# ztlpn/minilp

Measured on AMD Instinct MI355X. Metric: simplex pivots/sec, higher is better.
Workload: dtype f64; 1 GPU; config 4: random LP 100000 vars x 100000 constraints, 100 nnz/row (0.1% fill), Max c'x, Ax<=b, x>=0; primal simplex with PSE+DSE from the slack basis; timed pivots 5..1983; parallelism=1 GPU, nucleus_size_at_end=1559, completed_steps=1978

## Files before the change

include/minilp_hip.h:

```cpp
#ifndef MINILP_HIP_H
#define MINILP_HIP_H

#include <stdint.h>

#ifdef __cplusplus
extern "C" {
#endif

typedef struct mlp_problem mlp_problem;
typedef struct mlp_solution mlp_solution;

enum { MLP_MINIMIZE = 0, MLP_MAXIMIZE = 1 };
enum { MLP_EQ = 0, MLP_LE = 1, MLP_GE = 2 };
enum { MLP_OK = 0, MLP_INFEASIBLE = 1, MLP_UNBOUNDED = 2,
       MLP_EINVAL = -1, MLP_ESINGULAR = -2, MLP_EHIP = -3, MLP_ENOGPU = -4, MLP_ENOMEM = -5 };

#define MLP_ABI_VERSION 5u
uint32_t mlp_abi_version(void);
uint64_t mlp_stats_size(void);

const char* mlp_last_error(void);
int mlp_device_count(void);
int mlp_set_device(int device);

// ... 185 lines not shown
    int32_t phase;
    int32_t next_stage;
    int32_t reserved;
    int64_t col, row;
    int64_t entering_var, leaving_var;
    double pivot_coeff;
    double step;
    double objective;
    uint64_t nucleus_size;
} mlp_iter_info;
int mlp_engine_open(mlp_solution* s, mlp_iter_info* out);
int mlp_engine_stage(mlp_solution* s, int stage, mlp_iter_info* out);

double mlp_util_min_cut(uint32_t n, const double* weights, uint8_t* side_out);

#ifdef __cplusplus
}
#endif
#endif
```

minilp_amd/api.py:

```python
import ctypes as C
import os

import numpy as np

_HERE = os.path.dirname(os.path.abspath(__file__))
_SO = os.path.join(_HERE, "libminilp_hip.so")
os.environ.setdefault("HSA_ENABLE_IPC_MODE_LEGACY", "0")

MINIMIZE, MAXIMIZE = 0, 1
EQ, LE, GE = 0, 1, 2


class Infeasible(Exception):
    pass


class Unbounded(Exception):
    pass


class InternalError(Exception):
    def __init__(self, code, msg):
        super().__init__(f"[{code}] {msg}")
        self.code = code
# ... 131 lines not shown
    sig("mlp_solution_add_gomory_cut", i32, C.POINTER(vp), u32)
    sig("mlp_solution_stats", None, vp, C.POINTER(MlpStats))
    sig("mlp_solution_reset_stats", None, vp)
    sig("mlp_solution_trace_len", u64, vp)
    sig("mlp_solution_trace_get", None, vp, u64, C.POINTER(C.c_int32), C.POINTER(i64), C.POINTER(i64), C.POINTER(i64),
        C.POINTER(i64), pdbl, pdbl)
    sig("mlp_solution_state", u64, vp, C.c_char_p, pdbl, u64)
    sig("mlp_mps_parse", i32, C.c_char_p, u64, i32, C.POINTER(vp))
    sig("mlp_mps_free", None, vp)
    sig("mlp_mps_name", C.c_char_p, vp)
    sig("mlp_mps_num_vars", u32, vp)
    sig("mlp_mps_var_name", C.c_char_p, vp, u32)
    sig("mlp_mps_var_index", i64, vp, C.c_char_p)
    sig("mlp_mps_problem", vp, vp)
    sig("mlp_util_min_cut", C.c_double, u32, pdbl, C.POINTER(C.c_uint8))
    sig("mlp_solution_num_constraints", u64, vp)
    sig("mlp_solution_dual_values", i32, vp, pdbl, u64)
    sig("mlp_solution_dual_value", i32, vp, u64, pdbl)
    sig("mlp_solution_reduced_costs", i32, vp, pdbl, u32)
    sig("mlp_solution_reduced_cost", i32, vp, u32, pdbl)
    sig("mlp_solution_certificate", i32, vp, C.POINTER(MlpCertificate))
    sig("mlp_ranging_info_size", u64)
    if L.mlp_ranging_info_size() != C.sizeof(MlpRangingInfo):
        raise ImportError(f"{_SO}: mlp_ranging_info is {L.mlp_ranging_info_size()} bytes, this binding {C.sizeof(MlpRangingInfo)}: rebuild it")
    sig("mlp_solution_basis_status", i32, vp, C.POINTER(C.c_int32), u32, C.POINTER(C.c_int32), u64)
    sig("mlp_solution_cost_ranging", i32, vp, pu32, u64, pdbl, pdbl)
    sig("mlp_solution_rhs_ranging", i32, vp, C.POINTER(C.c_uint64), u64, pdbl, pdbl)
    sig("mlp_solution_ranging_info", i32, vp, C.POINTER(MlpRangingInfo))
    sig("mlp_cut_info_size", u64)
    if L.mlp_cut_info_size() != C.sizeof(MlpCutInfo):
# ... 79 lines not shown
    return idx, val


def _p(a, t):
    return a.ctypes.data_as(C.POINTER(t))


def min_cut(weights):
    w = np.ascontiguousarray(weights, dtype=np.float64)
    n = w.shape[0]
    side = np.zeros(n, dtype=np.uint8)
    val = lib().mlp_util_min_cut(n, _p(w, C.c_double), _p(side, C.c_uint8))
    return float(val), side.astype(bool)


class Problem:

    def __init__(self, direction, _h=None):
        self._h = _h if _h is not None else lib().mlp_problem_new(int(direction))
        self.direction = direction

    def __del__(self):
        if getattr(self, "_h", None):
            lib().mlp_problem_free(self._h)
            self._h = None

    def clone(self):
        return Problem(self.direction, lib().mlp_problem_clone(self._h))

    @property
# ... 425 lines not shown
```

minilp_amd/csrc/capi.hip:

```cpp
#include "../../include/minilp_hip.h"

#include <cmath>
#include <cstring>
#include <string>
#include <vector>

#include "engine.h"

using namespace mlp;


struct mlp_problem {
    ProblemData pd;
};
struct mlp_solution {
    Engine* eng = nullptr;
    bool duals_valid = false;
    Engine::Duals duals;
    Engine::RangingInfo ranging;
    Engine::CutInfo cuts;
    Engine::TableauInfo tableau;
    Engine::GmiInfo gmi;
    std::vector<uint64_t> tab_indptr;
    std::vector<uint32_t> tab_indices;
// ... 608 lines not shown
    s->eng->stats = Stats();
    s->eng->restart_sampling();
}
uint64_t mlp_solution_trace_len(const mlp_solution* s) { return s->eng->trace_log.size(); }
void mlp_solution_trace_get(const mlp_solution* s, uint64_t i, int32_t* phase, int64_t* col, int64_t* row,
                            int64_t* entering_var, int64_t* leaving_var, double* pivot_coeff, double* obj_after) {
    const PivotRecord& r = s->eng->trace_log[i];
    *phase = r.phase; *col = r.col; *row = r.row; *entering_var = r.entering_var; *leaving_var = r.leaving_var;
    *pivot_coeff = r.pivot_coeff; *obj_after = r.obj_after;
}
uint64_t mlp_solution_state(const mlp_solution* s, const char* what, double* out, uint64_t cap) {
    uint64_t n = (uint64_t)-1;
    guarded([&] { n = s->eng->state(what, out, cap); });
    return n;
}

int mlp_mps_parse(const char* text, uint64_t len, int direction, mlp_mps** out) {
    *out = nullptr;
    mlp_mps* f = new mlp_mps();
    int st = guarded([&] { f->d = parse_mps(std::string(text, len), direction == MLP_MAXIMIZE ? 1 : 0); });
    if (st != 0) delete f;
    else *out = f;
    return st;
}
void mlp_mps_free(mlp_mps* f) { delete f; }
const char* mlp_mps_name(const mlp_mps* f) { return f->d.name.c_str(); }
uint32_t mlp_mps_num_vars(const mlp_mps* f) { return (uint32_t)f->d.var_names.size(); }
const char* mlp_mps_var_name(const mlp_mps* f, uint32_t i) { return f->d.var_names[i].c_str(); }
int64_t mlp_mps_var_index(const mlp_mps* f, const char* name) {
    for (size_t i = 0; i < f->d.var_names.size(); ++i)
// ... 11 lines not shown
```

minilp_amd/csrc/engine.h:

```cpp
#pragma once
#include <hip/hip_runtime.h>

#include <cstdint>
#include <functional>
#include <utility>
#include <stdexcept>
#include <string>
#include <vector>

#include "kernels.h"

namespace mlp {

enum Stage { STAGE_FTRAN = 0, STAGE_RATIO = 1, STAGE_BTRAN = 2, STAGE_BASIS = 3, STAGE_ROW = 4, STAGE_APPLY = 5 };

struct MlpError : std::runtime_error {
    int code;
    MlpError(int c, const std::string& s) : std::runtime_error(s), code(c) {}
};
struct LpFail {
    int code;
};

#define HIPCHECK(expr)                                                                                   \
// ... 308 lines not shown
    DevBuf<unsigned char> d_pk_valid;
    DevBuf<unsigned char> d_fmark;
    bool use_pack = true;
    bool pack_built = false;
    size_t band_total_ = 0;
    bool use_order = true;
    uint64_t order_built_at = 0;
    uint64_t lifetime_pivots = 0;
    uint64_t order_every = 2048;
    bool order_valid = false;
    uint64_t order_from = 4096;
    bool order_force = false;
    void refresh_nb_order(bool force);
    int det_mode = -1;
    int banded_mode = -1;
    bool use_banded() const;
  public:
    bool banded_active() const { return use_banded(); }
    bool factor_active() const { return fac_on_; }
    void restart_sampling() { batches_run = 0; }
  private:
    void ensure_banded();
    DevBuf<int> d_fpk_cnt, d_fpk_var;
    DevBuf<double> d_fpk_val, d_fpk_x, d_fpk_part;
    DevBuf<unsigned char> d_fpk_in;
    bool fpull_on_ = true;
    bool fpk_valid_ = false;
    uint64_t fpk_built_at_ = 0, fpk_builds_ = 0;
    int fpk_every_ = 1024;
    bool fpk_wanted() const;
// ... 156 lines not shown
```

minilp_amd/csrc/engine.hip:

```cpp
#include "engine.h"


#include <algorithm>
#include <chrono>
#include <cmath>
#include <cstdio>
#include <cstdlib>
#include <climits>
#include <cstring>
#include <limits>
#include <map>
#include <memory>
#include <mutex>

#include <dlfcn.h>
#include <fcntl.h>
#include <sys/mman.h>
#include <sys/stat.h>
#include <unistd.h>

namespace mlp {

static const double INF = std::numeric_limits<double>::infinity();
static double now_s() {
// ... 39 lines not shown
    std::memset(&hview, 0, sizeof(hview));
    const char* ng = std::getenv("MLP_NO_GRAPH");
    use_graph = !(ng && ng[0] == '1');
    const char* rt = std::getenv("MLP_REFRESH_TOL");
    if (rt) refresh_tol = std::atof(rt);
    const char* lr = std::getenv("MLP_LOWRANK");
    if (lr) lr_force = std::max(0, std::min(LR_MAX, std::atoi(lr)));
    const char* lp = std::getenv("MLP_LDPAD");
    if (lp) ld_pad = std::max(0, std::min(4096, std::atoi(lp))) & ~1;
    const char* bt = std::getenv("MLP_BIGTILE");
    force_big_tiles = bt && std::atoi(bt) != 0;
    const char* dm = std::getenv("MLP_DETERMINISTIC");
    if (dm) det_mode = std::atoi(dm) != 0 ? 1 : 0;
    const char* bd = std::getenv("MLP_BANDED");
    if (bd) banded_mode = std::atoi(bd) != 0 ? 1 : 0;
    const char* fr = std::getenv("MLP_FINAL_REFRESH");
    if (fr) final_refresh_pivots = std::atol(fr);
    if (const char* sp = std::getenv("MLP_SWEEP_PACKED")) use_pack = sp[0] != '0';
    if (const char* of = std::getenv("MLP_ORDER_FROM")) order_from = (uint64_t)std::atoll(of);
    if (const char* oe = std::getenv("MLP_ORDER_EVERY")) order_every = (uint64_t)std::atoll(oe);
    const char* lz = std::getenv("MLP_LAZY_DSE");
    lazy_dse = !(lz && lz[0] == '0');
    ratio_two = std::getenv("MLP_RATIO_TWO_KERNELS") != nullptr;
    if (const char* hy = std::getenv("MLP_HYPER")) hyper_mode = std::atoi(hy) > 0 ? 1 : 0;
    if (const char* phk = std::getenv("MLP_PRIMAL_HEAD_K")) ph_kmax = std::max(0, std::atoi(phk));
    if (const char* sbk = std::getenv("MLP_SMALL_BASIS_K")) sb_kmax = std::max(0, std::min(256, std::atoi(sbk)));
    if (const char* sk = std::getenv("MLP_STR_K")) str_kmax = std::atoi(sk);
    if (const char* hh = std::getenv("MLP_HYPER_HEAVY")) hyper_heavy = std::atol(hh);
    if (const char* rs = std::getenv("MLP_RATIO_SPIN_LIMIT")) ratio_spin_limit = std::atoll(rs);
    if (const char* sb = std::getenv("MLP_STREAM_BALANCED")) sw_balanced = std::atoi(sb);
// ... 212 lines not shown
    const int lr = lr_force >= 0 ? lr_force : (cap_ >= 8192 ? 32 : 0);
    g.head_fused = (!fac_on_ && lr == 0 && max_col_nnz_ <= HEAD_LIST_CAP && max_row_nnz_ <= HEAD_LIST_CAP) ? 1 : 0;
    g.fac = fac_on_ ? 1 : 0;
    g.ratio_two = (ratio_two || (shard_world > 1 && ranks_share_device)) ? 1 : 0;
    g.ratio_list = ratio_spin_limit > 0 ? 1 : 0;
    g.str = (str_now && !stepping && !fac_on_) ? 1 : 0;
    g.sb = (g.str && sb_now) ? 1 : 0;
    g.ph = (g.str && ph_now) ? 1 : 0;
    g.fp = hview.fpk_on ? 1 : 0;
    return g;
}

bool Engine::use_banded() const {
    if (banded_mode == 0) return false;
    if (banded_mode == 1) return true;
    return m_ >= 4 * BAND_ROWS && h_rcol.size() >= ((size_t)1 << 22);
}
void Engine::ensure_banded() {
    if (!banded_dirty) return;
    const int nb = (m_ + BAND_ROWS - 1) / BAND_ROWS;
    const size_t np = (size_t)nb * (size_t)(N_ + 1);
    d_bptr.ensure(np, 0, st);
    d_scan_tmp.ensure(np / 4096 + 8, 0, st);
    launch_band_count(d_cptr.p, d_crow.p, N_, nb, d_bptr.p, st);
    launch_exclusive_scan(d_bptr.p, d_bptr.p, (long)np, d_scan_tmp.p, st);
    int total = 0;
    HIPCHECK(hipMemcpyAsync(&total, d_scan_tmp.p + (np + 4095) / 4096, sizeof(int), hipMemcpyDeviceToHost, st));
    HIPCHECK(hipStreamSynchronize(st));
    d_brow.ensure((size_t)total + 8, 0, st);
    d_bval.ensure((size_t)total + 8, 0, st);
    band_total_ = (size_t)total;
    pack_built = false;
    HIPCHECK(hipMemsetAsync(d_brow.p + total, 0, 8 * sizeof(unsigned short), st));
    HIPCHECK(hipMemsetAsync(d_bval.p + total, 0, 8 * sizeof(double), st));
    launch_band_fill(d_cptr.p, d_crow.p, d_cval.p, N_, nb, d_bptr.p, d_brow.p, d_bval.p, st);
    d_band_part.ensure((size_t)nb * (size_t)num_vars, 0, st);
    banded_dirty = false;
}

void Engine::refresh_nb_order(bool force) {
    if (!force && (!order_valid || lifetime_pivots - order_built_at < order_every)) return;
    std::vector<int> ord;
    ord.reserve((size_t)num_vars);
    for (int var = 0; var < N_; ++var)
        if (h_var_loc[var] < 0) ord.push_back(-1 - h_var_loc[var]);
    if ((int)ord.size() != num_vars) throw MlpError(-3, "refresh_nb_order: host mirror of var_loc is inconsistent");
    d_nb_order.ensure((size_t)num_vars, 0, st);
    HIPCHECK(hipMemcpyAsync(d_nb_order.p, ord.data(), sizeof(int) * (size_t)num_vars, hipMemcpyHostToDevice, st));
    HIPCHECK(hipStreamSynchronize(st));
    order_built_at = lifetime_pivots;
    order_valid = true;
    pack_built = false;
    if (use_pack && band_total_ > 0 && !banded_dirty) {
        const int nb = (m_ + BAND_ROWS - 1) / BAND_ROWS;
        const size_t np = (size_t)nb * ((size_t)num_vars + 1);
        try {
            d_pk_ptr.ensure(np, 0, st);
            {
                const unsigned short* r0 = d_pk_row.p;
                const double* v0 = d_pk_val.p;
                d_pk_row.ensure(band_total_ + 16, 0, st);
                d_pk_val.ensure(band_total_ + 16, 0, st);
                if (d_pk_row.p != r0) HIPCHECK(hipMemsetAsync(d_pk_row.p, 0, sizeof(unsigned short) * d_pk_row.cap, st));
                if (d_pk_val.p != v0) HIPCHECK(hipMemsetAsync(d_pk_val.p, 0, sizeof(double) * d_pk_val.cap, st));
            }
            d_pk_valid.ensure((size_t)num_vars, 0, st);
            d_scan_tmp.ensure(np / 4096 + 8, 0, st);
        } catch (MlpError&) {
            (void)hipGetLastError();
// ... 87 lines not shown
    v.det_pull = (!v.pb_on && (det_mode == 1 || shard_det || force_det_push_ || (det_mode < 0 && h_rcol.size() <= ((size_t)1 << 21)))) ? 1 : 0;
    if (v.det_pull) {
        const unsigned char* before = d_fmark.p;
        d_fmark.ensure((size_t)m_ + 64, 0, st);
        if (d_fmark.p != before) HIPCHECK(hipMemsetAsync(d_fmark.p, 0, d_fmark.cap, st));
        v.fmark = d_fmark.p;
    } else {
        v.fmark = nullptr;
    }
    v.banded = use_banded() ? 1 : 0;
    if (v.banded) ensure_banded();
    v.bptr = v.banded ? d_bptr.p : nullptr;
    v.brow = v.banded ? d_brow.p : nullptr;
    v.bval = v.banded ? d_bval.p : nullptr;
    v.band_part = v.banded ? d_band_part.p : nullptr;
    v.nbands = (m_ + BAND_ROWS - 1) / BAND_ROWS;
    if (v.banded && use_order && shard_world == 1 && (lifetime_pivots >= order_from || order_force)) {
        if (!order_valid || (use_pack && !pack_built)) refresh_nb_order(true);
        v.nb_order = d_nb_order.p;
    } else {
        v.nb_order = nullptr;
    }
    const bool pk = v.nb_order && use_pack && pack_built;
    v.pk_ptr = pk ? d_pk_ptr.p : nullptr; v.pk_row = pk ? d_pk_row.p : nullptr; v.pk_val = pk ? d_pk_val.p : nullptr;
    v.pk_valid = pk ? d_pk_valid.p : nullptr;
    v.pos_of_kslot = d_pos_of_kslot.p; v.row_of_kslot = d_row_of_kslot.p; v.W = d_W.p;
    v.U = d_U.p; v.V = d_V.p; v.Ut = d_Ut.p;
    v.lrJ = fac_on_ ? 0 : (lr_force >= 0 ? lr_force : (cap_ >= 8192 ? 32 : 0));
    v.alpha_q = d_work.p;
    v.tau = d_work.p + (size_t)m_;
    v.rv = reinterpret_cast<double2*>(d_work.p + 2 * (size_t)m_);
// ... 2696 lines not shown
    e->h_obj = h_obj; e->h_lo = h_lo; e->h_hi = h_hi; e->h_rhs = h_rhs;
    e->h_cons_row = h_cons_row;
    e->h_rptr = h_rptr; e->h_rcol = h_rcol; e->h_rval = h_rval;
    e->h_colnnz = h_colnnz; e->h_single_row = h_single_row; e->h_single_val = h_single_val;
    e->max_col_nnz_ = max_col_nnz_; e->max_row_nnz_ = max_row_nnz_; e->amax_ = amax_; e->fpull_on_ = fpull_on_;
    e->sw_balanced = sw_balanced; e->str_kmax = str_kmax; e->sb_kmax = sb_kmax; e->ph_kmax = ph_kmax; e->hyper_mode = hyper_mode; e->hyper_heavy = hyper_heavy; e->hyper_backoff_max = hyper_backoff_max; e->ratio_two = ratio_two; e->ratio_spin_limit = ratio_spin_limit; e->ranks_share_device = false; e->lazy_dse = lazy_dse; e->beta_stale = beta_stale; e->use_order = use_order; e->use_pack = use_pack; e->order_force = order_force; e->lifetime_pivots = lifetime_pivots;
    e->h_basic_vars = h_basic_vars; e->h_nb_vars = h_nb_vars; e->h_var_loc = h_var_loc;
    e->h_kslot_of_pos = h_kslot_of_pos; e->h_srow_of_pos = h_srow_of_pos; e->h_kslot_of_row = h_kslot_of_row;
    e->h_pos_of_srow = h_pos_of_srow; e->h_sdiag_of_pos = h_sdiag_of_pos; e->h_nb_fixed = h_nb_fixed;
    e->h_pos_of_kslot = h_pos_of_kslot; e->h_row_of_kslot = h_row_of_kslot;
    e->enable_pse = enable_pse; e->enable_dse = enable_dse;
    e->primal_feasible = primal_feasible; e->dual_feasible = dual_feasible;
    e->resume_in_optimize = resume_in_optimize;
    e->nnz_nonbasic = nnz_nonbasic;
    e->trace = trace; e->profile = profile;
    e->banded_mode = banded_mode; e->det_mode = det_mode;
    e->final_refresh_pivots = final_refresh_pivots; e->iters_since_recalc = iters_since_recalc;
    e->iters_since_polish = iters_since_polish;
    e->ld_pad = ld_pad; e->lr_force = lr_force; e->force_big_tiles = force_big_tiles;
    hipStream_t s2 = e->st;
    {
        const size_t nz = h_rcol.size();
        e->d_cptr.copy_from(d_cptr, (size_t)N_ + 1, s2); e->d_crow.copy_from(d_crow, nz, s2); e->d_cval.copy_from(d_cval, nz, s2);
        e->d_rptr.copy_from(d_rptr, (size_t)m_ + 1, s2); e->d_rcol.copy_from(d_rcol, nz, s2); e->d_rval.copy_from(d_rval, nz, s2);
        e->d_lo.copy_from(d_lo, (size_t)N_, s2); e->d_hi.copy_from(d_hi, (size_t)N_, s2); e->d_obj.copy_from(d_obj, (size_t)N_, s2);
        e->colblk_dirty = true;
        e->banded_dirty = true;
        e->view_dirty = true;
    }
    int mk = m_;
    e->m_ = 0;
// ... 80 lines not shown
    else if (w == "dev_csc_indices") from_dev_i(d_crow, h_rcol.size());
    else if (w == "dev_csc_data") from_dev_d(d_cval.p, h_rcol.size());
    else if (w == "dev_csr_indptr") from_dev_i(d_rptr, (size_t)m_ + 1);
    else if (w == "dev_csr_data") from_dev_d(d_rval.p, h_rcol.size());
    else if (w == "flags") tmp = {(double)primal_feasible, (double)dual_feasible, (double)enable_pse, (double)enable_dse};
    else if (w == "small_basis_launches") {
        pull_ctl();
        tmp = {(double)h_ctl->sb_count};
    } else if (w == "dual_list_tests") {
        int n_ = 0, p_ = 0;
        HIPCHECK(hipMemcpy(&n_, &d_ctl.p->ar_used, sizeof(int), hipMemcpyDeviceToHost));
        HIPCHECK(hipMemcpy(&p_, &d_ctl.p->ar_pauses, sizeof(int), hipMemcpyDeviceToHost));
        tmp = {(double)n_, (double)p_};
    } else if (w == "fpull") {
        tmp = {(double)(hview.fpk_on ? 1 : 0), (double)fpk_builds_, (double)fpk_built_at_, (double)(fpull_supported(hview, geom()) ? 1 : 0)};
    } else if (w == "ratio_primal_form") {
        tmp = {(double)ratio_primal_form(hview, geom())};
    } else if (w == "ratio_list") {
        pull_ctl();
        const Geom g_ = geom();
        tmp = {(double)((ratio_primal_form(hview, g_) == 1 && ratio_list_cap(hview, g_) >= 0) ? 1 : 0), (double)h_ctl->rl_decisions, (double)h_ctl->rl_overflows};
    } else if (w == "btran_ride") {
        pull_ctl();
        tmp = {(double)(btran_rides_ratio(hview, geom()) ? 1 : 0), (double)h_ctl->rk_rides};
    } else if (w == "golive_checks") {
        tmp = {(double)golive_checks_};
    } else if (w == "shard_live") {
        tmp = {(double)(shard_is_live() ? 1 : 0)};
    } else if (w == "primal_head_launches") {
        pull_ctl();
// ... 492 lines not shown
```

minilp_amd/csrc/kernels.h:

```cpp
#pragma once
#include <hip/hip_runtime.h>
#include <stdint.h>

namespace mlp {

constexpr double EPS = 1e-8;

enum IterStatus : int {
    ITER_PIVOT = 0,
    ITER_FLIP = 1,
    ITER_OPTIMAL = 2,
    ITER_UNBOUNDED = 3,
    ITER_FEASIBLE = 4,
    ITER_INFEASIBLE = 5,
    ITER_SINGULAR = 6,
    ITER_NONE = 7,
    ITER_COMM = 8,
    ITER_STALL = 9,
};

struct IterState {
    int status;
    int q;
    int r;
// ... 161 lines not shown
    int* srow_of_pos;
    double* sdiag_of_pos;
    int* kslot_of_row;
    int* pos_of_srow;
    RowInfo* rowinfo;
    int* colblk;
    double* push_part;
    int pb_rb, pb_on;
    int pb_det, pb_hbits;
    double pb_amax;
    int* bptr;
    unsigned short* brow;
    double* bval;
    double2* band_part;
    int nbands, banded;
    unsigned char* fmark;
    int det_pull;
    int* pos_of_kslot;
    int* row_of_kslot;
    double* W;
    double* U;
    double* Ut;
    double* V;
    int lrJ;
    int sw_nbal, sw_pad;
    int* hy_stamp_n;
    int* hy_stamp_p;
    int* hy_var_slot;
    int2* hy_brng;
    double* hy_score;
// ... 70 lines not shown
};
constexpr int FAC_BMAX = 1024;
constexpr int AR_CAP = 2048;
constexpr int RK_LDS = 64;
constexpr int RL_CAP = 8;
constexpr int RL_BLOCKS = 512;
constexpr int TK_ONE = 128;
constexpr int TK_GROUPS = 16;
constexpr int TK_STRIDE = 1024;
constexpr int TK_WORDS = TK_STRIDE * (TK_GROUPS + 1) + 8;
constexpr int FAC_BAR_FLAG = TK_WORDS + 1024;

constexpr int FW_TR = 8;
constexpr int FW_TC = 1024;

constexpr int BAND_ROWS = 8192;
constexpr int BAND_THREADS = 1024;
constexpr int PB_ROWS = 4096;
constexpr int PB_CHUNKS = 48;
constexpr int PB_CHUNKS_DEFAULT = 24;

struct Geom {
    int m, n, cap;
    int lanes;
    int sweep_one;
    int sweep_variant;
    int big;
    int head_fused;
    int str;
    int sb;
    int fac;
// ... 149 lines not shown
    double2* rv;
    int k, fac;
};
int tab_wt_stripes(int k);
void launch_tab_rows(const DevView& dv, const Geom& g, const RangingBufs& b, int nreq, const int* h_req, double* ad, int* cnt, int* off,
                     int* sums, int* len, double* rhs, hipStream_t st);
void launch_tab_rhs(const DevView& dv, const TabBufs& b, const int* req, int nreq, int mode, hipStream_t st);
void launch_tab_solve(const DevView& dv, const Geom& g, const TabBufs& b, int transpose, int nreq, hipStream_t st);
void launch_blocked_inverse(const DevView& dv, int k, double* rowbuf, int nrowbuf, int* piv, int* src, double* prow, double* ckey,
                            int* cidx, int* flag, hipStream_t st);

void launch_csc_append_rows(const int* optr, const int* orow, const double* oval, int n_old, int row0, int R, const int* rptr,
                            const int* rcol, const double* rval, int* cnt, int* sums, int* nptr, int* nrow, double* nval,
                            hipStream_t st);
void launch_exclusive_scan(const int* in, int* out, long n, int* sums, hipStream_t st);
void launch_band_count(const int* cptr, const int* crow, int N, int nbands, int* cnt, hipStream_t st);
void launch_pack_count(const DevView& dv, int* cnt, hipStream_t st);
void launch_pack_fill(const DevView& dv, const int* pkptr, unsigned short* prow, double* pval, unsigned char* valid, hipStream_t st);
void launch_band_fill(const int* cptr, const int* crow, const double* cval, int N, int nbands, const int* bptr, unsigned short* brow,
                      double* bval, hipStream_t st);
void launch_build_colblk(const int* cptr, const int* crow, int N, int rb, int* colblk, hipStream_t st);

}
```

minilp_amd/csrc/kernels.hip:

```cpp
#include "kernels.h"
#include <hip/hip_ext.h>

#include <limits.h>
#include <math.h>

#include <cstdlib>
#include <string>

namespace mlp {

#define NONE_IDX INT_MAX
constexpr int BLK = 256;

struct Cand {
    double key;
    int idx;
};
__device__ __forceinline__ Cand cand_none() { return Cand{-INFINITY, NONE_IDX}; }
__device__ __forceinline__ bool cand_better(const Cand& a, const Cand& b) {
    return a.key > b.key || (a.key == b.key && a.idx < b.idx);
}
__device__ __forceinline__ Cand wave_best(Cand c) {
#pragma unroll
    for (int o = 32; o > 0; o >>= 1) {
// ... 2466 lines not shown
            const int lane = threadIdx.x & 63, lead = __ffsll((long long)mask) - 1;
            int base = 0;
            if (lane == lead) base = atomicAdd(&c->ar_n, __popcll(mask));
            base = __shfl(base, lead, 64);
            if (nz) v.ar_list[base + __popcll(mask & ((1ull << lane) - 1ull))] = col;
        }
    }
}
typedef unsigned int uint4u __attribute__((ext_vector_type(4), aligned(4)));
typedef double dbl2u __attribute__((ext_vector_type(2), aligned(8)));
template <int MODE, bool VORD>
__global__ void __launch_bounds__(BAND_THREADS) k_sweep_band(DevView v, int chunks) {
    Ctl* c = v.ctl;
    if (c->halt || c->it.status != ITER_PIVOT) return;
    KMARK0(c, 22);
    extern __shared__ double2 s_rv[];
    const int n_band_blocks = v.nbands * chunks;
    if ((int)blockIdx.x >= n_band_blocks) {
        struct_update_body(v, c, ((int)blockIdx.x - n_band_blocks) * BAND_THREADS + threadIdx.x);
        return;
    }
    const int b = (int)blockIdx.x / chunks, chunk = (int)blockIdx.x % chunks, tid = threadIdx.x;
    const int row0 = b * BAND_ROWS;
    const int nrows = min(BAND_ROWS, v.m - row0);
    for (int t = tid; t < nrows; t += BAND_THREADS) s_rv[t] = v.rv[row0 + t];
    for (int t = nrows + tid; t < BAND_ROWS; t += BAND_THREADS) s_rv[t] = make_double2(0.0, 0.0);
    __syncthreads();
    const int base = VORD ? 0 : v.nb_lo;
    const int span = VORD ? v.m + v.n : v.nb_hi - v.nb_lo;
    const int per = (span + chunks - 1) / chunks;
    const int c_lo = base + chunk * per;
    const int c_hi = min(base + span, c_lo + per);
    const int* bp = v.bptr + (size_t)b * (size_t)(v.m + v.n + 1);
    double2* out = v.band_part + (size_t)b * (size_t)v.n;
    constexpr int CPT = 4;
    for (int j0 = c_lo + tid; j0 < c_hi; j0 += CPT * BAND_THREADS) {
    int vars[CPT], poss[CPT], begs[CPT], ends[CPT];
    bool pkd[CPT];
    const int* pkp = (!VORD && v.pk_ptr) ? v.pk_ptr + (size_t)b * (size_t)(v.n + 1) : nullptr;
#pragma unroll
    for (int u = 0; u < CPT; ++u) {
        const int i = j0 + u * BAND_THREADS;
// ... 38 lines not shown
        const double* __restrict__ Vl = pkd[u] ? v.pk_val : v.bval;
        double a1 = 0.0, a2 = 0.0;
        for (int e0 = beg; e0 < end; e0 += 8) {
            const uint4u rr = *reinterpret_cast<const uint4u*>(Rw + e0);
            const dbl2u x0 = *reinterpret_cast<const dbl2u*>(Vl + e0);
            const dbl2u x1 = *reinterpret_cast<const dbl2u*>(Vl + e0 + 2);
            const dbl2u x2 = *reinterpret_cast<const dbl2u*>(Vl + e0 + 4);
            const dbl2u x3 = *reinterpret_cast<const dbl2u*>(Vl + e0 + 6);
            const unsigned r[8] = {rr.x & 0xffffu, rr.x >> 16, rr.y & 0xffffu, rr.y >> 16,
                                   rr.z & 0xffffu, rr.z >> 16, rr.w & 0xffffu, rr.w >> 16};
            double a[8] = {x0.x, x0.y, x1.x, x1.y, x2.x, x2.y, x3.x, x3.y};
            const int nv = end - e0;
#pragma unroll
            for (int u = 1; u < 8; ++u)
                if (u >= nv) a[u] = 0.0;
#pragma unroll
            for (int u = 0; u < 8; ++u) {
                const double2 t = s_rv[r[u]];
                if (MODE != 2) a1 += a[u] * t.x;
                if (MODE != 0) a2 += a[u] * t.y;
            }
        }
        out[j] = make_double2(a1, a2);
    }
    }
}
template <int MODE>
__global__ void __launch_bounds__(BLK) k_band_combine(DevView v, int n_comb) {
    Ctl* c = v.ctl;
    if (c->halt || c->it.status != ITER_PIVOT) return;
    if ((int)blockIdx.x >= n_comb) {
        struct_update_body(v, c, ((int)blockIdx.x - n_comb) * BLK + threadIdx.x);
        return;
    }
    const int i = v.nb_lo + blockIdx.x * BLK + threadIdx.x;
// ... 1499 lines not shown
__global__ void __launch_bounds__(1024) k_scan_add(int* out, long n, const int* sums) {
    const long base = (long)blockIdx.x * SCAN_TILE + (long)threadIdx.x * 4;
    const int off = sums[blockIdx.x];
#pragma unroll
    for (int u = 0; u < 4; ++u)
        if (base + u < n) out[base + u] += off;
}
void launch_exclusive_scan(const int* in, int* out, long n, int* sums, hipStream_t st) {
    const int nb = (int)((n + SCAN_TILE - 1) / SCAN_TILE);
    hipLaunchKernelGGL(k_scan_blocks, dim3(nb), dim3(1024), 0, st, in, out, n, sums);
    hipLaunchKernelGGL(k_scan_sums, dim3(1), dim3(1024), 0, st, sums, nb);
    hipLaunchKernelGGL(k_scan_add, dim3(nb), dim3(1024), 0, st, out, n, (const int*)sums);
}

__global__ void __launch_bounds__(BLK) k_band_count(const int* __restrict__ cptr, const int* __restrict__ crow, int N, int nbands,
                                                     int* __restrict__ cnt) {
    const int var = blockIdx.x * BLK + threadIdx.x;
    if (var > N) return;
    if (var == N) {
        for (int b = 0; b < nbands; ++b) cnt[(size_t)b * (N + 1) + N] = 0;
        return;
    }
    int e = cptr[var];
    const int end = cptr[var + 1];
    for (int b = 0; b < nbands; ++b) {
        const int lim = (b + 1) * BAND_ROWS;
        int c = 0;
        while (e < end && crow[e] < lim) {
            ++e;
            ++c;
        }
        cnt[(size_t)b * (N + 1) + var] = (c + 1) & ~1;
    }
}
__global__ void __launch_bounds__(BLK) k_band_fill(const int* __restrict__ cptr, const int* __restrict__ crow,
                                                    const double* __restrict__ cval, int N, int nbands, const int* __restrict__ bptr,
                                                    unsigned short* __restrict__ brow, double* __restrict__ bval) {
    const int var = blockIdx.x * BLK + threadIdx.x;
    if (var >= N) return;
    int e = cptr[var];
    const int end = cptr[var + 1];
    for (int b = 0; b < nbands; ++b) {
        const int lim = (b + 1) * BAND_ROWS, row0 = b * BAND_ROWS;
        int dst = bptr[(size_t)b * (N + 1) + var];
        const int dend = bptr[(size_t)b * (N + 1) + var + 1];
        while (e < end && crow[e] < lim) {
            brow[dst] = (unsigned short)(crow[e] - row0);
            bval[dst] = cval[e];
            ++e;
            ++dst;
        }
        if (dst < dend) {
            brow[dst] = 0;
            bval[dst] = 0.0;
        }
    }
}
void launch_band_count(const int* cptr, const int* crow, int N, int nbands, int* cnt, hipStream_t st) {
    hipLaunchKernelGGL(k_band_count, dim3(blocks_for(N + 1)), dim3(BLK), 0, st, cptr, crow, N, nbands, cnt);
}
void launch_band_fill(const int* cptr, const int* crow, const double* cval, int N, int nbands, const int* bptr, unsigned short* brow,
                      double* bval, hipStream_t st) {
    hipLaunchKernelGGL(k_band_fill, dim3(blocks_for(N)), dim3(BLK), 0, st, cptr, crow, cval, N, nbands, bptr, brow, bval);
}
__global__ void __launch_bounds__(BLK) k_pack_count(DevView v, int* __restrict__ cnt) {
    const long g = (long)blockIdx.x * BLK + threadIdx.x;
    const int n1 = v.n + 1;
    if (g >= (long)v.nbands * n1) return;
    const int b = (int)(g / n1), i = (int)(g % n1);
    int len = 0;
    if (i < v.n) {
        const int var = v.nb_vars[v.nb_order[i]];
        const int* bp = v.bptr + (size_t)b * (size_t)(v.m + v.n + 1);
        len = bp[var + 1] - bp[var];
    }
    cnt[g] = len;
}
__global__ void __launch_bounds__(BLK) k_pack_fill(DevView v, const int* __restrict__ pkptr, unsigned short* __restrict__ prow,
// ... 456 lines not shown
    do {                                                                                                   \
        int n_rhs = with_rhs ? blocks_for((long)g.cap * G) : 0;                                            \
        hipLaunchKernelGGL(k_btran<G>, dim3(n_gather + n_rhs), dim3(BLK), 0, st, dv, n_gather, after_fold); \
    } while (0)
    LANES_SWITCH(g.lanes, BTRAN(4), BTRAN(16), BTRAN(64));
#undef BTRAN
}
void launch_btran_rhs(const DevView& dv, const Geom& g, hipStream_t st) {
    LANES_SWITCH(g.lanes,
                 hipLaunchKernelGGL(k_btran_rhs<4>, dim3(blocks_for((long)g.cap * 4)), dim3(BLK), 0, st, dv),
                 hipLaunchKernelGGL(k_btran_rhs<16>, dim3(blocks_for((long)g.cap * 16)), dim3(BLK), 0, st, dv),
                 hipLaunchKernelGGL(k_btran_rhs<64>, dim3(blocks_for((long)g.cap * 64)), dim3(BLK), 0, st, dv));
}
static void launch_sweep_banded(const DevView& dv, const Geom& g, int mode, int with_struct, int inline_combine, hipStream_t st) {
    static bool attr_set = false;
    const size_t lds = sizeof(double2) * (size_t)BAND_ROWS;
    if (!attr_set) {
        (void)hipFuncSetAttribute(reinterpret_cast<const void*>(k_sweep_band<0, false>), hipFuncAttributeMaxDynamicSharedMemorySize, (int)lds);
        (void)hipFuncSetAttribute(reinterpret_cast<const void*>(k_sweep_band<1, false>), hipFuncAttributeMaxDynamicSharedMemorySize, (int)lds);
        (void)hipFuncSetAttribute(reinterpret_cast<const void*>(k_sweep_band<2, false>), hipFuncAttributeMaxDynamicSharedMemorySize, (int)lds);
        (void)hipFuncSetAttribute(reinterpret_cast<const void*>(k_sweep_band<0, true>), hipFuncAttributeMaxDynamicSharedMemorySize, (int)lds);
        (void)hipFuncSetAttribute(reinterpret_cast<const void*>(k_sweep_band<1, true>), hipFuncAttributeMaxDynamicSharedMemorySize, (int)lds);
        (void)hipFuncSetAttribute(reinterpret_cast<const void*>(k_sweep_band<2, true>), hipFuncAttributeMaxDynamicSharedMemorySize, (int)lds);
        attr_set = true;
    }
    const bool vord = false;
    const int struct_blocks = (inline_combine && with_struct) ? (g.cap + BAND_THREADS - 1) / BAND_THREADS : 0;
    int chunks = (256 - struct_blocks) / dv.nbands;
    if (chunks < 1) chunks = 1;
    const dim3 gr(dv.nbands * chunks + struct_blocks), b(BAND_THREADS);
    if (vord) {
        if (mode == 0) LAUNCH_T(1, (k_sweep_band<0, true>), gr, b, lds, st, dv, chunks);
        else if (mode == 1) LAUNCH_T(1, (k_sweep_band<1, true>), gr, b, lds, st, dv, chunks);
        else LAUNCH_T(1, (k_sweep_band<2, true>), gr, b, lds, st, dv, chunks);
    } else {
        if (mode == 0) LAUNCH_T(1, (k_sweep_band<0, false>), gr, b, lds, st, dv, chunks);
        else if (mode == 1) LAUNCH_T(1, (k_sweep_band<1, false>), gr, b, lds, st, dv, chunks);
        else LAUNCH_T(1, (k_sweep_band<2, false>), gr, b, lds, st, dv, chunks);
// ... 374 lines not shown
```

Baseline: 11170 pivots/s.

## Use adaptive band height and compact LDS layout with nonzero-flag bitmap in banded sweep

Band height is now computed from m so that bands are balanced and at most 16384 rows each, replacing the fixed 8192-row bands, and it can be overridden by an environment variable. The banded sweep kernel now stages only one double per row in LDS plus a ballot-built bitmap marking rows where the other component is nonzero. In mode 1 it reads that second component from global memory only for flagged rows. This roughly halves LDS per row so larger bands fit and fewer bands need sweeping, at the cost of extra bitmap work and scattered global loads when the flagged component is dense. The change also adds a query API and exposes the geometry through the state interface.

```diff
diff --git a/include/minilp_hip.h b/include/minilp_hip.h
--- a/include/minilp_hip.h
+++ b/include/minilp_hip.h
@@ -223,6 +223,8 @@
 
 double mlp_util_min_cut(uint32_t n, const double* weights, uint8_t* side_out);
 
+void mlp_band_geometry(int64_t m, int32_t forced, int32_t* nbands, int32_t* band_rows);
+
 #ifdef __cplusplus
 }
 #endif
diff --git a/minilp_amd/api.py b/minilp_amd/api.py
--- a/minilp_amd/api.py
+++ b/minilp_amd/api.py
@@ -169,6 +169,7 @@
     sig("mlp_mps_var_index", i64, vp, C.c_char_p)
     sig("mlp_mps_problem", vp, vp)
     sig("mlp_util_min_cut", C.c_double, u32, pdbl, C.POINTER(C.c_uint8))
+    sig("mlp_band_geometry", None, i64, i32, C.POINTER(i32), C.POINTER(i32))
     sig("mlp_solution_num_constraints", u64, vp)
     sig("mlp_solution_dual_values", i32, vp, pdbl, u64)
     sig("mlp_solution_dual_value", i32, vp, u64, pdbl)
@@ -278,6 +279,12 @@
     return float(val), side.astype(bool)
 
 
+def band_geometry(m, forced=0):
+    nb, rows = C.c_int32(), C.c_int32()
+    lib().mlp_band_geometry(int(m), int(forced), C.byref(nb), C.byref(rows))
+    return nb.value, rows.value
+
+
 class Problem:
 
     def __init__(self, direction, _h=None):
diff --git a/minilp_amd/csrc/capi.hip b/minilp_amd/csrc/capi.hip
--- a/minilp_amd/csrc/capi.hip
+++ b/minilp_amd/csrc/capi.hip
@@ -646,6 +646,12 @@
     guarded([&] { n = s->eng->state(what, out, cap); });
     return n;
 }
+void mlp_band_geometry(int64_t m, int32_t forced, int32_t* nbands, int32_t* band_rows) {
+    int nb = 1, rows = 64;
+    band_geometry((int)std::max<int64_t>(0, std::min<int64_t>(m, INT32_MAX)), forced, &nb, &rows);
+    *nbands = nb;
+    *band_rows = rows;
+}
 
 int mlp_mps_parse(const char* text, uint64_t len, int direction, mlp_mps** out) {
     *out = nullptr;
diff --git a/minilp_amd/csrc/engine.h b/minilp_amd/csrc/engine.h
--- a/minilp_amd/csrc/engine.h
+++ b/minilp_amd/csrc/engine.h
@@ -346,6 +346,8 @@
     void refresh_nb_order(bool force);
     int det_mode = -1;
     int banded_mode = -1;
+    int band_rows_force = 0;
+    int band_rows_ = 0;
     bool use_banded() const;
   public:
     bool banded_active() const { return use_banded(); }
diff --git a/minilp_amd/csrc/engine.hip b/minilp_amd/csrc/engine.hip
--- a/minilp_amd/csrc/engine.hip
+++ b/minilp_amd/csrc/engine.hip
@@ -77,6 +77,7 @@
     if (dm) det_mode = std::atoi(dm) != 0 ? 1 : 0;
     const char* bd = std::getenv("MLP_BANDED");
     if (bd) banded_mode = std::atoi(bd) != 0 ? 1 : 0;
+    if (const char* br = std::getenv("MLP_BAND_ROWS")) band_rows_force = std::max(64, std::min(BAND_ROWS_MAX, std::atoi(br)));
     const char* fr = std::getenv("MLP_FINAL_REFRESH");
     if (fr) final_refresh_pivots = std::atol(fr);
     if (const char* sp = std::getenv("MLP_SWEEP_PACKED")) use_pack = sp[0] != '0';
@@ -319,15 +320,20 @@
 bool Engine::use_banded() const {
     if (banded_mode == 0) return false;
     if (banded_mode == 1) return true;
-    return m_ >= 4 * BAND_ROWS && h_rcol.size() >= ((size_t)1 << 22);
+    return m_ >= BANDED_MIN_ROWS && h_rcol.size() >= ((size_t)1 << 22);
 }
 void Engine::ensure_banded() {
     if (!banded_dirty) return;
-    const int nb = (m_ + BAND_ROWS - 1) / BAND_ROWS;
+    int nb = 1, rows = 64;
+    band_geometry(m_, band_rows_force, &nb, &rows);
+    if (rows != band_rows_) {
+        if (d_pk_row.p) HIPCHECK(hipMemsetAsync(d_pk_row.p, 0, sizeof(unsigned short) * d_pk_row.cap, st));
+        band_rows_ = rows;
+    }
     const size_t np = (size_t)nb * (size_t)(N_ + 1);
     d_bptr.ensure(np, 0, st);
     d_scan_tmp.ensure(np / 4096 + 8, 0, st);
-    launch_band_count(d_cptr.p, d_crow.p, N_, nb, d_bptr.p, st);
+    launch_band_count(d_cptr.p, d_crow.p, N_, nb, rows, d_bptr.p, st);
     launch_exclusive_scan(d_bptr.p, d_bptr.p, (long)np, d_scan_tmp.p, st);
     int total = 0;
     HIPCHECK(hipMemcpyAsync(&total, d_scan_tmp.p + (np + 4095) / 4096, sizeof(int), hipMemcpyDeviceToHost, st));
@@ -338,7 +344,7 @@
     pack_built = false;
     HIPCHECK(hipMemsetAsync(d_brow.p + total, 0, 8 * sizeof(unsigned short), st));
     HIPCHECK(hipMemsetAsync(d_bval.p + total, 0, 8 * sizeof(double), st));
-    launch_band_fill(d_cptr.p, d_crow.p, d_cval.p, N_, nb, d_bptr.p, d_brow.p, d_bval.p, st);
+    launch_band_fill(d_cptr.p, d_crow.p, d_cval.p, N_, nb, rows, d_bptr.p, d_brow.p, d_bval.p, st);
     d_band_part.ensure((size_t)nb * (size_t)num_vars, 0, st);
     banded_dirty = false;
 }
@@ -357,7 +363,8 @@
     order_valid = true;
     pack_built = false;
     if (use_pack && band_total_ > 0 && !banded_dirty) {
-        const int nb = (m_ + BAND_ROWS - 1) / BAND_ROWS;
+        int nb = 1, rows = 64;
+        band_geometry(m_, band_rows_force, &nb, &rows);
         const size_t np = (size_t)nb * ((size_t)num_vars + 1);
         try {
             d_pk_ptr.ensure(np, 0, st);
@@ -475,7 +482,8 @@
     v.brow = v.banded ? d_brow.p : nullptr;
     v.bval = v.banded ? d_bval.p : nullptr;
     v.band_part = v.banded ? d_band_part.p : nullptr;
-    v.nbands = (m_ + BAND_ROWS - 1) / BAND_ROWS;
+    band_geometry(m_, band_rows_force, &v.nbands, &v.band_rows);
+    v.pad6 = 0;
     if (v.banded && use_order && shard_world == 1 && (lifetime_pivots >= order_from || order_force)) {
         if (!order_valid || (use_pack && !pack_built)) refresh_nb_order(true);
         v.nb_order = d_nb_order.p;
@@ -3202,7 +3210,7 @@
     e->resume_in_optimize = resume_in_optimize;
     e->nnz_nonbasic = nnz_nonbasic;
     e->trace = trace; e->profile = profile;
-    e->banded_mode = banded_mode; e->det_mode = det_mode;
+    e->banded_mode = banded_mode; e->band_rows_force = band_rows_force; e->det_mode = det_mode;
     e->final_refresh_pivots = final_refresh_pivots; e->iters_since_recalc = iters_since_recalc;
     e->iters_since_polish = iters_since_polish;
     e->ld_pad = ld_pad; e->lr_force = lr_force; e->force_big_tiles = force_big_tiles;
@@ -3313,6 +3321,10 @@
         tmp = {(double)n_, (double)p_};
     } else if (w == "fpull") {
         tmp = {(double)(hview.fpk_on ? 1 : 0), (double)fpk_builds_, (double)fpk_built_at_, (double)(fpull_supported(hview, geom()) ? 1 : 0)};
+    } else if (w == "band_geometry") {
+        int nb = 1, rows = 64;
+        band_geometry(m_, band_rows_force, &nb, &rows);
+        tmp = {(double)nb, (double)rows};
     } else if (w == "ratio_primal_form") {
         tmp = {(double)ratio_primal_form(hview, geom())};
     } else if (w == "ratio_list") {
diff --git a/minilp_amd/csrc/kernels.h b/minilp_amd/csrc/kernels.h
--- a/minilp_amd/csrc/kernels.h
+++ b/minilp_amd/csrc/kernels.h
@@ -199,6 +199,7 @@
     double* bval;
     double2* band_part;
     int nbands, banded;
+    int band_rows, pad6;
     unsigned char* fmark;
     int det_pull;
     int* pos_of_kslot;
@@ -299,7 +300,20 @@
 constexpr int FW_TR = 8;
 constexpr int FW_TC = 1024;
 
-constexpr int BAND_ROWS = 8192;
+constexpr int BAND_ROWS_MAX = 16384;
+constexpr int BANDED_MIN_ROWS = 32768;
+inline void band_geometry(int m, int forced, int* nbands, int* band_rows) {
+    int rows;
+    if (forced > 0) {
+        rows = (forced < 64 ? 64 : forced > BAND_ROWS_MAX ? BAND_ROWS_MAX : forced);
+        rows = (rows + 63) & ~63;
+    } else {
+        const int nb = m > 0 ? (m + BAND_ROWS_MAX - 1) / BAND_ROWS_MAX : 1;
+        rows = ((m > 0 ? (m + nb - 1) / nb : 1) + 63) & ~63;
+    }
+    *band_rows = rows;
+    *nbands = m > 0 ? (m + rows - 1) / rows : 1;
+}
 constexpr int BAND_THREADS = 1024;
 constexpr int PB_ROWS = 4096;
 constexpr int PB_CHUNKS = 48;
@@ -479,11 +493,11 @@
                             const int* rcol, const double* rval, int* cnt, int* sums, int* nptr, int* nrow, double* nval,
                             hipStream_t st);
 void launch_exclusive_scan(const int* in, int* out, long n, int* sums, hipStream_t st);
-void launch_band_count(const int* cptr, const int* crow, int N, int nbands, int* cnt, hipStream_t st);
+void launch_band_count(const int* cptr, const int* crow, int N, int nbands, int band_rows, int* cnt, hipStream_t st);
 void launch_pack_count(const DevView& dv, int* cnt, hipStream_t st);
 void launch_pack_fill(const DevView& dv, const int* pkptr, unsigned short* prow, double* pval, unsigned char* valid, hipStream_t st);
-void launch_band_fill(const int* cptr, const int* crow, const double* cval, int N, int nbands, const int* bptr, unsigned short* brow,
-                      double* bval, hipStream_t st);
+void launch_band_fill(const int* cptr, const int* crow, const double* cval, int N, int nbands, int band_rows, const int* bptr,
+                      unsigned short* brow, double* bval, hipStream_t st);
 void launch_build_colblk(const int* cptr, const int* crow, int N, int rb, int* colblk, hipStream_t st);
 
 }
diff --git a/minilp_amd/csrc/kernels.hip b/minilp_amd/csrc/kernels.hip
--- a/minilp_amd/csrc/kernels.hip
+++ b/minilp_amd/csrc/kernels.hip
@@ -2504,18 +2504,36 @@
     Ctl* c = v.ctl;
     if (c->halt || c->it.status != ITER_PIVOT) return;
     KMARK0(c, 22);
-    extern __shared__ double2 s_rv[];
+    extern __shared__ double s_x[];
+    const int BR = v.band_rows;
+    unsigned long long* s_flag = reinterpret_cast<unsigned long long*>(s_x + BR);
     const int n_band_blocks = v.nbands * chunks;
     if ((int)blockIdx.x >= n_band_blocks) {
         struct_update_body(v, c, ((int)blockIdx.x - n_band_blocks) * BAND_THREADS + threadIdx.x);
         return;
     }
     const int b = (int)blockIdx.x / chunks, chunk = (int)blockIdx.x % chunks, tid = threadIdx.x;
-    const int row0 = b * BAND_ROWS;
-    const int nrows = min(BAND_ROWS, v.m - row0);
-    for (int t = tid; t < nrows; t += BAND_THREADS) s_rv[t] = v.rv[row0 + t];
-    for (int t = nrows + tid; t < BAND_ROWS; t += BAND_THREADS) s_rv[t] = make_double2(0.0, 0.0);
+    const int row0 = b * BR;
+    const int nrows = min(BR, v.m - row0);
+    constexpr int FILL_U = 8;
+    for (int t0 = tid; t0 < BR; t0 += FILL_U * BAND_THREADS) {
+        double2 x[FILL_U];
+#pragma unroll
+        for (int i = 0; i < FILL_U; ++i) x[i] = v.rv[row0 + min(t0 + i * BAND_THREADS, nrows - 1)];
+#pragma unroll
+        for (int i = 0; i < FILL_U; ++i) {
+            const int t = t0 + i * BAND_THREADS;
+            if (t >= BR) break;
+            if (t >= nrows) x[i] = make_double2(0.0, 0.0);
+            s_x[t] = MODE == 0 ? x[i].x : x[i].y;
+            if (MODE == 1) {
+                const unsigned long long f = __ballot(x[i].x != 0.0);
+                if ((tid & 63) == 0) s_flag[t >> 6] = f;
+            }
+        }
+    }
     __syncthreads();
+    const unsigned* s_flag32 = reinterpret_cast<const unsigned*>(s_flag);
     const int base = VORD ? 0 : v.nb_lo;
     const int span = VORD ? v.m + v.n : v.nb_hi - v.nb_lo;
     const int per = (span + chunks - 1) / chunks;
@@ -2584,11 +2602,30 @@
 #pragma unroll
             for (int u = 1; u < 8; ++u)
                 if (u >= nv) a[u] = 0.0;
-#pragma unroll
-            for (int u = 0; u < 8; ++u) {
-                const double2 t = s_rv[r[u]];
-                if (MODE != 2) a1 += a[u] * t.x;
-                if (MODE != 0) a2 += a[u] * t.y;
+            if (MODE == 1) {
+                unsigned fw[8];
+                double rx[8], sx[8];
+#pragma unroll
+                for (int u = 0; u < 8; ++u) {
+                    fw[u] = s_flag32[r[u] >> 5];
+                    sx[u] = s_x[r[u]];
+                }
+#pragma unroll
+                for (int u = 0; u < 8; ++u) {
+                    rx[u] = 0.0;
+                    if (u < nv && ((fw[u] >> (r[u] & 31u)) & 1u)) rx[u] = v.rv[row0 + (int)r[u]].x;
+                }
+#pragma unroll
+                for (int u = 0; u < 8; ++u) {
+                    a1 += a[u] * rx[u];
+                    a2 += a[u] * sx[u];
+                }
+            } else {
+#pragma unroll
+                for (int u = 0; u < 8; ++u) {
+                    if (MODE == 0) a1 += a[u] * s_x[r[u]];
+                    else a2 += a[u] * s_x[r[u]];
+                }
             }
         }
         out[j] = make_double2(a1, a2);
@@ -4118,7 +4155,7 @@
 }
 
 __global__ void __launch_bounds__(BLK) k_band_count(const int* __restrict__ cptr, const int* __restrict__ crow, int N, int nbands,
-                                                     int* __restrict__ cnt) {
+                                                     int band_rows, int* __restrict__ cnt) {
     const int var = blockIdx.x * BLK + threadIdx.x;
     if (var > N) return;
     if (var == N) {
@@ -4128,7 +4165,7 @@
     int e = cptr[var];
     const int end = cptr[var + 1];
     for (int b = 0; b < nbands; ++b) {
-        const int lim = (b + 1) * BAND_ROWS;
+        const int lim = (b + 1) * band_rows;
         int c = 0;
         while (e < end && crow[e] < lim) {
             ++e;
@@ -4138,14 +4175,15 @@
     }
 }
 __global__ void __launch_bounds__(BLK) k_band_fill(const int* __restrict__ cptr, const int* __restrict__ crow,
-                                                    const double* __restrict__ cval, int N, int nbands, const int* __restrict__ bptr,
-                                                    unsigned short* __restrict__ brow, double* __restrict__ bval) {
+                                                    const double* __restrict__ cval, int N, int nbands, int band_rows,
+                                                    const int* __restrict__ bptr, unsigned short* __restrict__ brow,
+                                                    double* __restrict__ bval) {
     const int var = blockIdx.x * BLK + threadIdx.x;
     if (var >= N) return;
     int e = cptr[var];
     const int end = cptr[var + 1];
     for (int b = 0; b < nbands; ++b) {
-        const int lim = (b + 1) * BAND_ROWS, row0 = b * BAND_ROWS;
+        const int lim = (b + 1) * band_rows, row0 = b * band_rows;
         int dst = bptr[(size_t)b * (N + 1) + var];
         const int dend = bptr[(size_t)b * (N + 1) + var + 1];
         while (e < end && crow[e] < lim) {
@@ -4160,12 +4198,12 @@
         }
     }
 }
-void launch_band_count(const int* cptr, const int* crow, int N, int nbands, int* cnt, hipStream_t st) {
-    hipLaunchKernelGGL(k_band_count, dim3(blocks_for(N + 1)), dim3(BLK), 0, st, cptr, crow, N, nbands, cnt);
-}
-void launch_band_fill(const int* cptr, const int* crow, const double* cval, int N, int nbands, const int* bptr, unsigned short* brow,
-                      double* bval, hipStream_t st) {
-    hipLaunchKernelGGL(k_band_fill, dim3(blocks_for(N)), dim3(BLK), 0, st, cptr, crow, cval, N, nbands, bptr, brow, bval);
+void launch_band_count(const int* cptr, const int* crow, int N, int nbands, int band_rows, int* cnt, hipStream_t st) {
+    hipLaunchKernelGGL(k_band_count, dim3(blocks_for(N + 1)), dim3(BLK), 0, st, cptr, crow, N, nbands, band_rows, cnt);
+}
+void launch_band_fill(const int* cptr, const int* crow, const double* cval, int N, int nbands, int band_rows, const int* bptr,
+                      unsigned short* brow, double* bval, hipStream_t st) {
+    hipLaunchKernelGGL(k_band_fill, dim3(blocks_for(N)), dim3(BLK), 0, st, cptr, crow, cval, N, nbands, band_rows, bptr, brow, bval);
 }
 __global__ void __launch_bounds__(BLK) k_pack_count(DevView v, int* __restrict__ cnt) {
     const long g = (long)blockIdx.x * BLK + threadIdx.x;
@@ -4652,14 +4690,15 @@
 }
 static void launch_sweep_banded(const DevView& dv, const Geom& g, int mode, int with_struct, int inline_combine, hipStream_t st) {
     static bool attr_set = false;
-    const size_t lds = sizeof(double2) * (size_t)BAND_ROWS;
+    const size_t lds_max = sizeof(double) * (size_t)BAND_ROWS_MAX + (size_t)BAND_ROWS_MAX / 8;
+    const size_t lds = sizeof(double) * (size_t)dv.band_rows + (size_t)dv.band_rows / 8;
     if (!attr_set) {
-        (void)hipFuncSetAttribute(reinterpret_cast<const void*>(k_sweep_band<0, false>), hipFuncAttributeMaxDynamicSharedMemorySize, (int)lds);
-        (void)hipFuncSetAttribute(reinterpret_cast<const void*>(k_sweep_band<1, false>), hipFuncAttributeMaxDynamicSharedMemorySize, (int)lds);
-        (void)hipFuncSetAttribute(reinterpret_cast<const void*>(k_sweep_band<2, false>), hipFuncAttributeMaxDynamicSharedMemorySize, (int)lds);
-        (void)hipFuncSetAttribute(reinterpret_cast<const void*>(k_sweep_band<0, true>), hipFuncAttributeMaxDynamicSharedMemorySize, (int)lds);
-        (void)hipFuncSetAttribute(reinterpret_cast<const void*>(k_sweep_band<1, true>), hipFuncAttributeMaxDynamicSharedMemorySize, (int)lds);
-        (void)hipFuncSetAttribute(reinterpret_cast<const void*>(k_sweep_band<2, true>), hipFuncAttributeMaxDynamicSharedMemorySize, (int)lds);
+        (void)hipFuncSetAttribute(reinterpret_cast<const void*>(k_sweep_band<0, false>), hipFuncAttributeMaxDynamicSharedMemorySize, (int)lds_max);
+        (void)hipFuncSetAttribute(reinterpret_cast<const void*>(k_sweep_band<1, false>), hipFuncAttributeMaxDynamicSharedMemorySize, (int)lds_max);
+        (void)hipFuncSetAttribute(reinterpret_cast<const void*>(k_sweep_band<2, false>), hipFuncAttributeMaxDynamicSharedMemorySize, (int)lds_max);
+        (void)hipFuncSetAttribute(reinterpret_cast<const void*>(k_sweep_band<0, true>), hipFuncAttributeMaxDynamicSharedMemorySize, (int)lds_max);
+        (void)hipFuncSetAttribute(reinterpret_cast<const void*>(k_sweep_band<1, true>), hipFuncAttributeMaxDynamicSharedMemorySize, (int)lds_max);
+        (void)hipFuncSetAttribute(reinterpret_cast<const void*>(k_sweep_band<2, true>), hipFuncAttributeMaxDynamicSharedMemorySize, (int)lds_max);
         attr_set = true;
     }
     const bool vord = false;
```

Result: slower. 10550 pivots/s (-5.6%).
